# raphaelsulzer/PixelsPointsPolygons

Hardware: AMD Instinct MI355X
Metric: training tiles/sec (224px img + 3k-pt lidar) (higher is better)
Workload: dtype f32 (products as bf16x3 on the bf16 MFMA, fp32 accumulate); 1 GPU; pix2poly_fusion_s8_bs64x1; tiles_per_gpu=64, points_per_tile=3000, hip_graph=True, sync_bn=False, decoder_dropout=reference defaults (0.1 / 0.05), step=fwd+CE+10*BCE+bwd+AdamW, parallelism=dp1

## Files before the change

include/p3hip.h:

```cpp
#ifndef P3HIP_H
#define P3HIP_H
#include <stdint.h>

#ifdef __cplusplus
extern "C" {
#endif

#define P3_OK 0
#define P3_EINVAL (-1)
#define P3_ESHAPE (-2)
#define P3_EALIGN (-3)
#define P3_EUNSUP (-4)

#define P3_F32 0
#define P3_BF16 1
#define P3_F32X3 2

#define P3_ACT_NONE 0
#define P3_ACT_GELU 1
#define P3_ACT_RELU 2
#define P3_ACT_MUL 3
#define P3_ACT_BN_RELU 4

#define P3_A_PLAIN 0
#define P3_A_CONV3X3 1
#define P3_A_AFFINE_RELU 2
#define P3_A_PAIR_AFFINE_RELU 3
#define P3_A_AFFINE_MASK2 5
#define P3_A_CONV3X3_AFFINE_RELU 4

int p3_version(void);
const char* p3_last_error_string(void);
void p3_trace_kernels(int on);
const char* p3_last_kernel(void);

int p3_set_deterministic(void* scratch, int64_t bytes, int all_dtypes);
int p3_get_deterministic(void);
int p3_scratch_regions(int n);
int p3_scratch_side_stream(void* stream);
int p3_reduce_defer(float* arena, int64_t floats);
int p3_reduce_defer_enable(int on);
int p3_reduce_flush(void* stream);
int p3_reduce_pending(void);
int p3_reduce_drop(void);
int p3_scratch_stream(void* stream);
int p3_tn_defer(float* arena, int64_t floats);
int p3_tn_defer_enable(int on);
int p3_tn_flush(void* stream);
int p3_tn_pending(void);
int p3_tn_drop(void);

typedef struct {
    const unsigned long long* seed;
    unsigned int site;
    float p;
} p3_dropout;
int p3_rng_advance(unsigned long long* seed, void* stream);
int p3_transpose_many(const void* src, void* dst, const void* table, int n_entries, int total_tiles, void* stream);
int p3_dropout_apply(const void* in, int dtype_in, void* out, int dtype_out, int64_t n, int64_t ncols, const p3_dropout* drop, void* stream);

typedef struct {
    int M, N, K;
    int lda, ldb, ldc;
    int dtype_in;
    int dtype_out;
    int act;
    int a_mode;
    const float* bias;
    const void* residual;
    int ldr;
    int dtype_res;
    void* aux;
    int conv_H, conv_W, conv_C;
    const float* a_scale;
    const float* a_shift;
    const void* pair_V;
    int pair_n;
    float* colsum;
    float* colsumsq;
    p3_dropout drop;
    const void* bwd_saved;
    int bwd_act;
    float bwd_scale;
    int aux_mode;
    int conv_pad;
    const float* bwd_bn;
    const void* w_lo;
} p3_gemm_desc;
int p3_gemm(const void* A, const void* W, void* C, const p3_gemm_desc* d, void* stream);
int p3_gemm_dma(const void* A, const void* W, void* C, const p3_gemm_desc* d, int variant, void* stream);

typedef struct {
    int M, N, K;
    const void* a_hi; const void* a_lo; int lda;
    const void* w_hi; const void* w_lo; int ldb;
    void* c; void* c_lo; int ldc;
    const float* bias;
    const float* residual; int ldr;
    int act;
    float* aux; int ldaux;
    const float* mul; int ldmul;
    int tile;
    int conv_B, conv_H, conv_W, conv_ci, conv_row0;
} p3_gemm_x3_desc;
int p3_gemm_x3(const p3_gemm_x3_desc* d, void* stream);
int p3_gemm_x3_tile(int mode);
int p3_gemm_tn_x3(const void* a_hi, const void* a_lo, int lda, const void* b_hi, const void* b_lo, int ldb, float* C, int ldc, int M, int N, int K,
                  float* colsum, float* slabs, int max_slabs, void* stream);
int p3_gemm_tn_x3_conv(const void* a_hi, const void* a_lo, int lda, const void* b_hi, const void* b_lo, int ldb, float* C, int ldc, int M, int N, int Ci, int Pw,
                       float* slabs, int max_slabs, void* stream);
int p3_pad_nhwc_planes(const float* src, int ld_src, const float* pre, int ld_pre, const float* a, const float* b, void* hi, void* lo, int ld_dst, int B, int H,
                       int W, int C, int Cp, int guard, int64_t rows_total, void* stream);
int p3_col_stats(const float* x, int ld, int64_t M, int N, float* sums, float* scratch, int64_t scratch_floats, void* stream);
int p3_gemm_tn_x3_wide(int on);
int p3_to_planes(const float* src, int ld_src, void* hi, void* lo, int ld_dst, int64_t rows, int cols, void* stream);
int p3_from_planes(const void* hi, const void* lo, int ld_src, float* dst, int ld_dst, int64_t rows, int cols, void* stream);

int p3_layernorm(const void* x, const float* gamma, const float* beta, void* y, int64_t rows, int cols, int ldx, int ldy,
                 float eps, int dtype_in, int dtype_out, float* save_mean, float* save_rstd, void* stream);
int p3_layernorm_bwd_res(const void* dy, const void* x, const float* gamma, const float* mean, const float* rstd, const void* dres,
                         void* dx, float* dgamma, float* dbeta, int64_t rows, int cols, int dtype_dy, int dtype_x, int dtype_dx,
                         void* stream);
int p3_layernorm_bwd_lo(const void* dy, const void* x, const float* gamma, const float* mean, const float* rstd, const void* dres,
                        void* dx, void* dx_lo, float* dgamma, float* dbeta, int64_t rows, int cols, int dtype_dy, int dtype_x, int dtype_dx,
                        void* stream);
int p3_layernorm_bwd_lo_drop(const void* dy, const void* x, const float* gamma, const float* mean, const float* rstd, const void* dres,
                             void* dx, void* dx_lo, const p3_dropout* lo_drop, float* dgamma, float* dbeta, int64_t rows, int cols,
                             int dtype_dy, int dtype_x, int dtype_dx, void* stream);
int p3_layernorm_planes(const float* x, const float* gamma, const float* beta, void* y_hi, void* y_lo, int64_t rows, int cols, int ldx, int ldy, float eps,
                        float* save_mean, float* save_rstd, void* stream);
int p3_layernorm_bwd_planes(const float* dy, const float* x, const float* gamma, const float* mean, const float* rstd, const float* dres, float* dx,
                            void* dx_hi, void* dx_lo, int ld_planes, float* dgamma, float* dbeta, int64_t rows, int cols, void* stream);
int p3_layernorm_bwd(const void* dy, const void* x, const float* gamma, const float* mean, const float* rstd, void* dx,
                     float* dgamma, float* dbeta, int64_t rows, int cols, int dtype_dy, int dtype_x, int dtype_dx,
                     void* stream);

typedef struct {
    int B, H, Lq, Lk, head_dim;
    int64_t q_bs, k_bs, v_bs, o_bs;
    int q_rs, k_rs, v_rs, o_rs;
    float scale;
    int causal;
    const float* key_bias;
    int dtype;
    float* lse;
    p3_dropout drop;
    unsigned int* drop_rows;
    int grad_planes;
    int g_rs;
    int64_t g_bs, g_lo;
    void* o_planes;
    int op_rs;
    int64_t op_bs, op_lo;
} p3_attn_desc;
int p3_attention(const void* Q, const void* K, const void* V, void* O, const p3_attn_desc* d, void* stream);



typedef struct {
    int B;
    int64_t total_points;
    int nx, ny;
    float vx, vy, vz;
    float zmax;
    int max_points;
    int max_voxels;
    int C;
    int training;
    float bn_eps, bn_momentum;
    int dtype;
    int out_ld, out_col_off;
    int no_backward;
} p3_pillar_desc;
int64_t p3_pillar_stem_workspace_bytes(const p3_pillar_desc* d);
int p3_pillar_stem(const float* values, const int64_t* offsets, const float* w1, const float* bn1_gamma,
                   const float* bn1_beta, float* bn1_rmean, float* bn1_rvar, const void* w2, const float* bn2_gamma,
                   const float* bn2_beta, float* bn2_rmean, float* bn2_rvar, void* out, void* workspace,
                   const p3_pillar_desc* d, void* stream);
int p3_pillar_stem_layout(const p3_pillar_desc* d, int64_t* offsets);
int p3_pillar_stem_phased(const float* values, const int64_t* offsets, const float* w1, const float* bn1_gamma,
                          const float* bn1_beta, float* bn1_rmean, float* bn1_rvar, const void* w2, const float* bn2_gamma,
                          const float* bn2_beta, float* bn2_rmean, float* bn2_rvar, void* out, void* workspace,
                          const p3_pillar_desc* d, int phases, void* stream);
int p3_pillar_stem_bwd(const void* dcanvas, int dcanvas_ld, const float* w1, const float* bn1_gamma, const void* w2t,
                       const float* bn2_gamma, void* workspace, const p3_pillar_desc* d, float* dw1, float* dg1, float* db1,
                       float* dw2, float* dg2, float* db2, void* stream);
int p3_pillar_stem_bwd_phased(const void* dcanvas, int dcanvas_ld, const float* w1, const float* bn1_gamma, const void* w2t,
                              const float* bn2_gamma, void* workspace, const p3_pillar_desc* d, float* dw1, float* dg1, float* db1,
                              float* dw2, float* dg2, float* db2, const float* stat2, const float* stat1, int phases, void* stream);

int p3_patchify(const float* img, void* out, int B, int Cin, int H, int W, int P, int dtype_out, void* stream);
int p3_patchify_ld(const float* img, void* out, int B, int Cin, int H, int W, int P, int ldk, int dtype_out, void* stream);
int p3_posembed_resample(const float* table, const float* wy, const float* wx, float* out, int n_in, int n_out, int D, void* stream);
int p3_posembed_resample_bwd(const float* dout, const float* wy, const float* wx, float* dtable, int n_in, int n_out, int D, void* stream);
int p3_layerscale_fold(const float* gamma, const float* W, const float* b, float* Wf, float* bf, int N, int K, void* stream);
int p3_layerscale_fold_bwd(const float* gamma, const float* W, const float* b, const float* dWf, const float* dbf, float* dW, float* db,
                           float* dgamma, int N, int K, void* stream);
int p3_tokens_assemble(const void* src, int src_ld, int dtype_src, const float* scale, const float* shift, const float* cls,
                       const float* pos, float* x, int B, int np, int D, void* stream);
int p3_pool_pos(const void* y, int dtype_in, const float* pos, void* out, void* out_nopos, int dtype_out, int B, int np, int Din,
                int Dout, void* stream);
int p3_embed_tokens(const int64_t* tokens, const float* emb, const float* pos, void* x, float* key_bias, int B, int L, int D,
                    int pad_idx, int dtype_out, void* stream);
int p3_pair_mean(const void* feats, void* out, int B, int L, int N, int D, int dtype, void* stream);
int p3_pair_stats(const void* U, const void* V, int B, int N, int C, int dtype, float* sums, void* stream);
int p3_bn_finalize(const float* sums, int C, float count, const float* gamma, const float* beta, float* running_mean,
                   float* running_var, float eps, float momentum, int training, float* scale, float* shift, float* save_mean,
                   float* save_rstd, void* stream);
int p3_score_out(const void* H3, int dtype, const float* scale, const float* shift, const float* w4, const float* b4, float* out,
                 int B, int N, int C, int transpose_accumulate, void* stream);
int p3_sinkhorn(const float* scores, const float* alpha, int B, int m, int n, int iters, float* perm, float* z_full,
                float* uv_hist, void* stream);
int p3_assignment(const float* scores, int B, int N, int maximize, int32_t* col4row, float* perm, int32_t* status, void* stream);
int p3_argmax(const float* x, int64_t* out, int rows, int cols, int ld, void* stream);

typedef struct {
    int B, t, steps, Lmem;
    int D, H, FF;
    const void* x_in;  long long x_in_stride;
    void* x_out;       long long x_out_stride;
    void* kv_self;
    const void* kv_mem;
    const float* key_bias; long long key_bias_stride;
    const void* w_in;  const float* b_in;
    const void* w_so;  const float* b_so;
    const void* w_q;   const float* b_q;
    const void* w_co;  const float* b_co;
    const void* w1;    const float* b1;
    const void* w2;    const float* b2;
    const float *g1, *be1, *g2, *be2, *g3, *be3;
    float eps, scale;
    int cluster;
    float* exch;
    unsigned int* sync;
    int* err;
    int fp32;
} p3_decode_layer_desc;
int p3_decode_layer(const p3_decode_layer_desc* d, void* stream);
int p3_cast(const void* a, int dtype_a, void* b, int dtype_b, int64_t n, void* stream);
int p3_add_pos(const void* x, const float* pos, void* out, int B, int L, int D, int dtype, void* stream);

int p3_attention_bwd(const void* Q, const void* K, const void* V, const void* O, const void* dO, const float* lse, void* dQ,
                     void* dK, void* dV, float* delta_ws, const p3_attn_desc* d, void* stream);
int p3_gemm_tn(const void* A, const void* B, float* C, int M, int N, int K, int lda, int ldb, int ldc, int dtype, void* stream);
int p3_colsum(const void* x, float* out, int64_t M, int N, int ld, int dtype, void* stream);
int p3_act_bwd(const void* dy, int dtype_dy, const void* saved, int dtype_saved, void* out, int dtype_out, int64_t n, int act, float scale,
               void* stream);
int p3_embed_tokens_bwd(const void* dx, int dtype, const int64_t* tokens, float* demb, float* dpos, int B, int L, int D, void* stream);
int p3_embed_tokens_bwd_v(const void* dx, int dtype, const int64_t* tokens, float* demb, int B, int L, int D, int V, void* stream);
int p3_tokens_assemble_bwd(const float* dx, const void* src, int src_ld, int dtype_src, const float* scale, const float* shift, const float* mean,
                           void* dsrc, float* dscale, float* dshift, int B, int np, int D, void* stream);
int p3_pool_pos_bwd(const void* dout, int dtype_dout, void* dy, int dtype_dy, int B, int np, int Din, int Dout, void* stream);
int p3_pair_mean_bwd(const float* dF, void* dfeats, int dtype, int B, int L, int N, int D, int accumulate, void* stream);
int p3_sinkhorn_bwd(const float* scores, const float* alpha, int B, int m, int n, int iters, const float* perm,
                    const float* uv_hist, const float* dperm, float* dscores, float* dalpha, void* workspace, void* stream);
int64_t p3_sinkhorn_bwd_workspace_bytes(int B, int m, int n, int iters);
int p3_ce_loss_fwd(const float* logits, int ld, const int64_t* targets, int R, int V, int ignore_index, float* row_lse, float* acc, void* stream);
int p3_ce_loss_bwd(const float* logits, int ld, const int64_t* targets, int R, int V, int ignore_index, const float* row_lse,
                   const float* acc, const float* gscale, void* dlogits, int dtype_out, int ld_out, int Vpad, void* stream);
int p3_bce_loss_fwd(const float* p, const float* y, int64_t n, float* acc, void* stream);
int p3_bce_loss_bwd(const float* p, const float* y, int64_t n, const float* gscale, float* dp, void* stream);
int p3_adamw_schedule(long long* step, float* hyper, float base_lr, int kind, int warmup_steps, int total_steps, float beta1, float beta2,
                      void* stream);
int p3_adamw_schedule_dev(long long* step, float* hyper, const float* sched, float beta1, float beta2, void* stream);
int p3_adamw(float* params, const float* grads, float* exp_avg, float* exp_avg_sq, int64_t n, const float* hyper, float beta1,
             float beta2, float eps, float weight_decay, float grad_scale, void* bf16_shadow, void* stream);

// ... 139 lines not shown
```

pixelspointspolygons_amd/csrc/gemm_tn.hip:

```cpp
#include <stdio.h>
#include <stdlib.h>

#include <type_traits>

#include "p3_common.h"

namespace {

constexpr int TN = 128, TK = 128;

struct TnArgs {
    const void* A; const void* B; float* C;
    int M, N, K, lda, ldb, ldc, rows_per_split, tiles_k, splits;
    int Kb;
    int b_mode;
    const float* b_scale; const float* b_shift; const void* pair_V; int pair_n;
    float* slabs;
    float* colsum;
    float* cs_slab;
};

template <typename T> struct TTr;
template <> struct TTr<bf16_t> { static constexpr int BM = 64, PITCH = 160, ELEMS = 64 * 160; };
template <> struct TTr<float> { static constexpr int BM = 16, PITCH = 132, ELEMS = 16 * 132; };
// ... 350 lines not shown
            const float4 raw = *reinterpret_cast<const float4*>(p);
            a[0] += raw.x; a[1] += raw.y; a[2] += raw.z; a[3] += raw.w;
        }
    };
    if (c0 < N) {
        int64_t r = r0 + ry;
        for (; r + 3 * nrl < r1; r += 4 * nrl) {
            const T* p = x + r * ld + c0;
            add(p); add(p + (int64_t)nrl * ld); add(p + (int64_t)2 * nrl * ld); add(p + (int64_t)3 * nrl * ld);
        }
        for (; r < r1; r += nrl) add(x + r * ld + c0);
    }
#pragma unroll
    for (int k = 0; k < 4; ++k) red[ry * (ncq * 4) + q * 4 + k] = a[k];
    __syncthreads();
    if ((int)threadIdx.x < ncq * 4) {
        float s = 0.f;
        for (int y = 0; y < nrl; ++y) s += red[y * (ncq * 4) + threadIdx.x];
        const int c = blockIdx.y * 256 + threadIdx.x;
        if (c < N) {
            if (slab) slab[(int64_t)blockIdx.x * N + c] = s;
            else atomicAdd(out + c, s);
        }
    }
}

template <typename T>
__global__ __launch_bounds__(256) void colsum_scalar_kernel(const T* __restrict__ x, float* __restrict__ out, int64_t M, int N, int ld, int rows_per_block,
                                                            float* __restrict__ slab) {
    const int64_t r0 = (int64_t)blockIdx.x * rows_per_block;
    const int64_t r1 = r0 + rows_per_block < M ? r0 + rows_per_block : M;
    for (int c = threadIdx.x + blockIdx.y * 256; c < N; c += 256 * gridDim.y) {
        float s = 0.f;
        for (int64_t r = r0; r < r1; ++r) s += Cvt<T>::to_f(x[r * ld + c]);
        if (slab) slab[(int64_t)blockIdx.x * N + c] = s;
        else atomicAdd(out + c, s);
    }
}

}

void p3_tn_reduce_launch(const float* slabs, float* C, int N, int K, int ldc, int splits, hipStream_t s) {
    int64_t gr = ((int64_t)N * K + 255) / 256; if (gr > 4096) gr = 4096;
    hipLaunchKernelGGL(tn_reduce_kernel, dim3((int)gr), dim3(256), 0, s, slabs, C, N, K, ldc, splits);
}

namespace {
constexpr int TNP_MAX = 96;
struct TnpEntry { const float* slab; float* C; int N, K, ldc, splits, first_block, pad; };
struct TnpTable { TnpEntry e[TNP_MAX]; int n; };
constexpr int TNP_CAP = 4 * TNP_MAX;
TnpEntry g_tnp[TNP_CAP];
int g_tnp_n = 0, g_tnp_on = 0;
float* g_tnp_arena = nullptr;
int64_t g_tnp_cap = 0, g_tnp_used = 0;

__global__ __launch_bounds__(256) void tn_flush_kernel(TnpTable t) {
    int e = 0;
    while (e + 1 < t.n && (int)blockIdx.x >= t.e[e + 1].first_block) ++e;
    const TnpEntry en = t.e[e];
    const int64_t total = (int64_t)en.N * en.K;
    const int64_t i0 = ((int64_t)(blockIdx.x - en.first_block) * 256 + threadIdx.x) * 4;
    if (i0 >= total) return;
    double a[4] = {0.0, 0.0, 0.0, 0.0};
    int s = 0;
    for (; s + 8 <= en.splits; s += 8) {
        float4 v[8];
#pragma unroll
        for (int u = 0; u < 8; ++u) v[u] = *reinterpret_cast<const float4*>(en.slab + (int64_t)(s + u) * total + i0);
#pragma unroll
        for (int u = 0; u < 8; ++u) { a[0] += (double)v[u].x; a[1] += (double)v[u].y; a[2] += (double)v[u].z; a[3] += (double)v[u].w; }
    }
    for (; s < en.splits; ++s) {
        const float4 v = *reinterpret_cast<const float4*>(en.slab + (int64_t)s * total + i0);
        a[0] += (double)v.x; a[1] += (double)v.y; a[2] += (double)v.z; a[3] += (double)v.w;
    }
    const int n = (int)(i0 / en.K), k = (int)(i0 - (int64_t)n * en.K);
    float* c = en.C + (int64_t)n * en.ldc + k;
#pragma unroll
    for (int q = 0; q < 4; ++q) c[q] = (float)((double)c[q] + a[q]);
}
}

extern "C" int p3_tn_defer(float* arena, int64_t floats) { g_tnp_arena = arena; g_tnp_cap = arena ? floats : 0; g_tnp_used = 0; g_tnp_n = 0; return P3_OK; }
extern "C" int p3_tn_defer_enable(int on) { const int was = g_tnp_on; g_tnp_on = on ? 1 : 0; return was; }
extern "C" int p3_tn_pending(void) { return g_tnp_n; }
extern "C" int p3_tn_drop(void) { const int n = g_tnp_n; g_tnp_n = 0; g_tnp_used = 0; return n; }

float* p3_tn_park(float* C, int N, int K, int ldc, int splits) {
    const int64_t floats = (int64_t)splits * N * K;
    if (!g_tnp_on || !g_tnp_arena || g_tnp_n >= TNP_CAP || g_tnp_used + floats > g_tnp_cap || K % 4 != 0 || ldc % 4 != 0 || ((uintptr_t)C % 16) != 0) return nullptr;
    {
        const uintptr_t lo = (uintptr_t)C, hi = (uintptr_t)(C + (int64_t)(N - 1) * ldc + K);
        for (int i = 0; i < g_tnp_n; ++i) {
            const TnpEntry& o = g_tnp[i];
            const uintptr_t olo = (uintptr_t)o.C, ohi = (uintptr_t)(o.C + (int64_t)(o.N - 1) * o.ldc + o.K);
            if (lo < ohi && olo < hi) {
                if (o.ldc == ldc) {
                    const bool fwd = C >= o.C;
                    const int64_t dist = fwd ? C - o.C : o.C - C;
                    const int64_t cs = dist % ldc;
                    const int k_first = fwd ? o.K : K, k_second = fwd ? K : o.K;
                    if (cs >= k_first && cs + k_second <= ldc) continue;
                }
                return nullptr;
            }
        }
    }
    float* slot = g_tnp_arena + g_tnp_used;
    g_tnp_used += (floats + 63) / 64 * 64;
    TnpEntry& en = g_tnp[g_tnp_n++];
    en.slab = slot; en.C = C; en.N = N; en.K = K; en.ldc = ldc; en.splits = splits; en.first_block = 0; en.pad = 0;
    return slot;
}

extern "C" int p3_tn_flush(void* stream) {
    hipStream_t s = (hipStream_t)stream;
    for (int base = 0; base < g_tnp_n; base += TNP_MAX) {
        TnpTable t;
        t.n = g_tnp_n - base < TNP_MAX ? g_tnp_n - base : TNP_MAX;
        int blocks = 0;
        for (int i = 0; i < t.n; ++i) {
            t.e[i] = g_tnp[base + i];
            t.e[i].first_block = blocks;
            blocks += p3_ceil_div((int64_t)t.e[i].N * t.e[i].K, 1024);
        }
        hipLaunchKernelGGL(tn_flush_kernel, dim3(blocks), dim3(256), 0, s, t);
    }
    g_tnp_n = 0; g_tnp_used = 0;
    P3_LAUNCH_CHECK();
    return P3_OK;
}

extern "C" int p3_gemm_tn_ex(const void* A, const void* B, float* C, int M, int N, int K, int lda, int ldb, int ldc, int dtype_in, int b_mode,
                             const float* b_scale, const float* b_shift, const void* pair_V, int pair_n, float* colsum, float* slabs, int max_slabs, void* stream) {
    const bool split = dtype_in == P3_F32X3;
    const int dtype = split ? P3_F32 : dtype_in;
    P3_CHECK(A && B && C && M > 0 && N > 0 && K > 0, P3_EINVAL, "p3_gemm_tn: bad arguments");
    P3_CHECK(b_mode == 0 || b_mode == P3_A_AFFINE_RELU || b_mode == P3_A_PAIR_AFFINE_RELU || b_mode == P3_A_AFFINE_MASK2, P3_EINVAL, "p3_gemm_tn: b_mode");
    P3_CHECK(b_mode != P3_A_AFFINE_MASK2 || ldc >= 2 * K, P3_ESHAPE, "p3_gemm_tn: P3_A_AFFINE_MASK2 writes [N, 2K]");
    P3_CHECK(b_mode != P3_A_AFFINE_MASK2 || K % 8 == 0, P3_ESHAPE, "p3_gemm_tn: P3_A_AFFINE_MASK2 needs K % 8 == 0 (a staged vector must not straddle the two generated operands)");
    P3_CHECK(b_mode == 0 || (b_scale && b_shift), P3_EINVAL, "p3_gemm_tn: generated B operand needs b_scale / b_shift");
    P3_CHECK(b_mode != P3_A_PAIR_AFFINE_RELU || (pair_V && pair_n > 0 && M % (pair_n * pair_n) == 0), P3_ESHAPE, "p3_gemm_tn: pair mode needs V and M == B*n*n");
    P3_CHECK(dtype == P3_F32 || dtype == P3_BF16, P3_EUNSUP, "p3_gemm_tn: dtype");
    const int vec = dtype == P3_BF16 ? 8 : 4;
    P3_CHECK(N % vec == 0 && K % vec == 0 && lda % vec == 0 && ldb % vec == 0, P3_EALIGN, "p3_gemm_tn: N, K, lda, ldb must be multiples of 8 (bf16) / 4 (f32)");
    P3_CHECK(((uintptr_t)A % 16) == 0 && ((uintptr_t)B % 16) == 0, P3_EALIGN, "p3_gemm_tn: 16-byte base alignment");
    {
        const bool bf = dtype == P3_BF16, gen = (bf || split) && !colsum;
        hipStream_t hs = (hipStream_t)stream;
        int rc = P3_SKIP;
        if (bf && b_mode == 0)
            rc = p3_gemm_tn_dma_try(A, B, C, M, N, K, lda, ldb, ldc, colsum, slabs, max_slabs, hs);
        else if (gen && b_mode == P3_A_PAIR_AFFINE_RELU)
            rc = (bf ? p3_pair_dw_try : p3_pair_dw_x3_try)(A, B, C, M, N, K, lda, ldb, ldc, b_scale, b_shift, pair_V, pair_n, slabs, max_slabs, hs);
        else if (gen && b_mode == P3_A_AFFINE_MASK2)
            rc = (bf ? p3_mask2_dw_try : p3_mask2_dw_x3_try)(A, B, C, M, N, K, lda, ldb, ldc, b_scale, b_shift, slabs, max_slabs, hs);
        if (rc != P3_SKIP) return rc;
    }
    TnArgs g; g.A = A; g.B = B; g.C = C; g.M = M; g.N = N; g.K = K; g.lda = lda; g.ldb = ldb; g.ldc = ldc;
    g.Kb = K;
    if (b_mode == P3_A_AFFINE_MASK2) { K *= 2; g.K = K; }
    g.b_mode = b_mode; g.b_scale = b_scale; g.b_shift = b_shift; g.pair_V = pair_V; g.pair_n = pair_n; g.colsum = colsum;
    const int tiles_n = p3_ceil_div(N, TN);
    g.tiles_k = p3_ceil_div(K, TK);
    const int tiles = tiles_n * g.tiles_k;
    const int bm = dtype == P3_BF16 ? 64 : 16;
    const int tgt = 448;
    int splits = (512 % tiles == 0) ? 512 / tiles : p3_ceil_div(tgt, tiles);
    if (tgt <= 512 && splits > 1 && splits * tiles > 512) --splits;
    if (slabs && splits > max_slabs) splits = max_slabs;
    int max_splits = p3_ceil_div(M, 4 * bm);
    if (splits > max_splits) splits = max_splits;
    if (splits < 1) splits = 1;
    g.rows_per_split = p3_ceil_div(p3_ceil_div(M, splits), bm) * bm;
    splits = p3_ceil_div(M, g.rows_per_split);
    g.slabs = (slabs && splits > 1) ? slabs : nullptr;
    bool parked = false;
    if (g.slabs) { float* slot = p3_tn_park(C, N, K, ldc, splits); if (slot) { g.slabs = slot; parked = true; } }
    g.splits = splits;
    int cs_parked = 0;
    g.cs_slab = colsum ? p3_colsum_parts(splits, N, colsum, dtype, &cs_parked) : nullptr;
    dim3 grid(tiles * splits), block(256);
    hipStream_t s = (hipStream_t)stream;
#define P3_TN_LAUNCH(MODE)                                                                            \
    do {                                                                                              \
        if (dtype == P3_BF16) hipLaunchKernelGGL((gemm_tn_kernel<bf16_t, MODE>), grid, block, 0, s, g); \
        else if (split) hipLaunchKernelGGL((gemm_tn_kernel<float, MODE, true>), grid, block, 0, s, g); \
        else hipLaunchKernelGGL((gemm_tn_kernel<float, MODE>), grid, block, 0, s, g);                  \
    } while (0)
    if (p3_tracing()) {
        char nm[64];
        snprintf(nm, sizeof(nm), "gemm_tn_kernel<%s, %d>", dtype == P3_BF16 ? "bf16" : "float", g.b_mode);
        p3_note_kernel(nm);
    }
    if (g.b_mode == 0) P3_TN_LAUNCH(0);
    else if (g.b_mode == P3_A_AFFINE_RELU) P3_TN_LAUNCH(P3_A_AFFINE_RELU);
    else if (g.b_mode == P3_A_AFFINE_MASK2) P3_TN_LAUNCH(P3_A_AFFINE_MASK2);
    else P3_TN_LAUNCH(P3_A_PAIR_AFFINE_RELU);
#undef P3_TN_LAUNCH
    if (g.slabs && !parked) {
        int64_t gr = ((int64_t)N * K + 255) / 256; if (gr > 4096) gr = 4096;
        hipLaunchKernelGGL(tn_reduce_kernel, dim3((int)gr), dim3(256), 0, s, g.slabs, C, N, K, ldc, splits);
    }
    P3_LAUNCH_CHECK();
    if (g.cs_slab && !cs_parked) return p3_det_reduce(g.cs_slab, splits, N, colsum, N, 1, s);
    return P3_OK;
}

extern "C" int p3_gemm_tn(const void* A, const void* B, float* C, int M, int N, int K, int lda, int ldb, int ldc, int dtype, void* stream) {
    return p3_gemm_tn_ex(A, B, C, M, N, K, lda, ldb, ldc, dtype, 0, nullptr, nullptr, nullptr, 0, nullptr, nullptr, 0, stream);
}

extern "C" int p3_colsum(const void* x, float* out, int64_t M, int N, int ld, int dtype, void* stream) {
    P3_CHECK(x && out && M >= 0 && N > 0, P3_EINVAL, "p3_colsum: bad arguments");
    P3_CHECK(dtype == P3_BF16 || dtype == P3_F32, P3_EUNSUP, "p3_colsum: dtype");
    if (M == 0) return P3_OK;
    hipStream_t s = (hipStream_t)stream;
    const int es = dtype == P3_BF16 ? 2 : 4;
    const bool vec = (N % 4 == 0) && (ld % 4 == 0) && ((uintptr_t)x % (4 * es) == 0);
    int rpb = M > 16384 ? 128 : (M > 2048 ? 32 : 8);
    if (vec) {
        int ncq = 64;
        if (N < 256) { const int nq = (N + 3) / 4; ncq = 1; while (ncq < nq) ncq <<= 1; }
        const int cols_blocks = p3_ceil_div(N, 256);
        const int64_t want = 2048 / cols_blocks > 0 ? 2048 / cols_blocks : 1;
        const int64_t r = (M + want - 1) / want;
        if (r > rpb) rpb = (int)r;
        dim3 grid(p3_ceil_div(M, rpb), cols_blocks), block(256);
        float* slab = p3_det_scratch((int64_t)grid.x * N, dtype);
        if (dtype == P3_BF16) hipLaunchKernelGGL((colsum_kernel<bf16_t>), grid, block, 0, s, (const bf16_t*)x, out, M, N, ld, rpb, ncq, slab);
        else hipLaunchKernelGGL((colsum_kernel<float>), grid, block, 0, s, (const float*)x, out, M, N, ld, rpb, ncq, slab);
        P3_LAUNCH_CHECK();
        if (slab) return p3_det_reduce(slab, (int)grid.x, N, out, N, 1, s);
        return P3_OK;
    }
    dim3 grid(p3_ceil_div(M, rpb), p3_ceil_div(N, 256)), block(256);
    float* slab = p3_det_scratch((int64_t)grid.x * N, dtype);
    {
        if (dtype == P3_BF16) hipLaunchKernelGGL((colsum_scalar_kernel<bf16_t>), grid, block, 0, s, (const bf16_t*)x, out, M, N, ld, rpb, slab);
        else hipLaunchKernelGGL((colsum_scalar_kernel<float>), grid, block, 0, s, (const float*)x, out, M, N, ld, rpb, slab);
    }
    P3_LAUNCH_CHECK();
    if (slab) return p3_det_reduce(slab, (int)grid.x, N, out, N, 1, s);
    return P3_OK;
}
```

pixelspointspolygons_amd/csrc/p3_common.h:

```cpp
#pragma once
#include <hip/hip_runtime.h>
#include <stdint.h>
#include <stdio.h>
#include <string.h>
#include <type_traits>

#include "../../include/p3hip.h"
#include "gfx950_asm.h"

typedef uint16_t bf16_t;

typedef float f32x16 __attribute__((ext_vector_type(16)));
typedef float f32x4 __attribute__((ext_vector_type(4)));
typedef short s16x8 __attribute__((ext_vector_type(8)));
typedef short s16x4 __attribute__((ext_vector_type(4)));

__device__ __forceinline__ float bf2f(bf16_t v) { return __uint_as_float(((uint32_t)v) << 16); }
typedef float p3_f32x2 __attribute__((ext_vector_type(2)));
typedef __bf16 p3_bf16x2 __attribute__((ext_vector_type(2)));
__device__ __forceinline__ bf16_t f2bf(float f) { return __builtin_bit_cast(bf16_t, (__bf16)f); }
__device__ __forceinline__ uint32_t pack_bf2(float lo, float hi) {
    const p3_f32x2 f = {lo, hi};
    return __builtin_bit_cast(uint32_t, __builtin_convertvector(f, p3_bf16x2));
}
// ... 47 lines not shown
        const T s = red[i];
        tot = MAX ? (s > tot ? s : tot) : tot + s;
        if (i < w) base = MAX ? (s > base ? s : base) : base + s;
    }
    __syncthreads();
    total = tot;
    if (w == 0) return v;
    return MAX ? (base > v ? base : v) : base + v;
}

__device__ __forceinline__ uint32_t p3_hash32(uint32_t x) {
    x ^= x >> 16; x *= 0x7feb352du; x ^= x >> 15; x *= 0x846ca68bu; x ^= x >> 16;
    return x;
}
struct DropKey { uint32_t k0, k1, thresh; float inv_keep; bool on; };
__device__ __forceinline__ DropKey drop_key(const p3_dropout& dr) {
    DropKey k; k.on = dr.seed != nullptr && dr.p > 0.f; k.k0 = 0; k.k1 = 0; k.thresh = 0; k.inv_keep = 1.f;
    if (k.on) {
        const unsigned long long s = *dr.seed;
        k.k0 = p3_hash32((uint32_t)s ^ (dr.site * 0x9E3779B9u));
        k.k1 = p3_hash32((uint32_t)(s >> 32) + dr.site * 0x85EBCA6Bu + 0x1234567u);
        k.thresh = (uint32_t)(dr.p * 65536.f + 0.5f);
        if (k.thresh > 65535u) k.thresh = 65535u;
        k.inv_keep = 65536.f / (float)(65536u - k.thresh);
    }
    return k;
}
__device__ __forceinline__ uint32_t drop_rowkey(const DropKey& k, uint64_t row) {
    return (uint32_t)row * 0x9E3779B1u + (uint32_t)(row >> 32) * 0x7FEB352Du + k.k0;
}
__device__ __forceinline__ uint32_t drop_colkey(const DropKey& k, uint32_t col) { return (col >> 1) * 0x85EBCA77u + k.k1; }
__device__ __forceinline__ uint32_t drop_bits(uint32_t rowkey, uint32_t colkey) { return p3_hash32(rowkey ^ colkey); }
__device__ __forceinline__ bool drop_keep_lo(const DropKey& k, uint32_t bits) { return (bits & 0xffffu) >= k.thresh; }
__device__ __forceinline__ bool drop_keep_hi(const DropKey& k, uint32_t bits) { return (bits >> 16) >= k.thresh; }
__device__ __forceinline__ bool drop_keep(const DropKey& k, uint64_t row, uint32_t col) {
    const uint32_t bits = drop_bits(drop_rowkey(k, row), drop_colkey(k, col));
    return (col & 1u) ? drop_keep_hi(k, bits) : drop_keep_lo(k, bits);
}

__device__ __forceinline__ int xcd_remap(int bid, int nwg) {
    const int q = nwg / 8, r = nwg % 8, xcd = bid % 8, idx = bid / 8;
    return (xcd < r ? xcd * (q + 1) : r * (q + 1) + (xcd - r) * q) + idx;
}

__device__ __forceinline__ void attn_block_of(int lid, int nblk, int L, int pairs, int mode, int& blk, int& pair) {
    if (mode == 1 && nblk > 1 && (L & 127) != 0 && (pairs & 7) == 0) {
        const int p8 = pairs >> 3, per_xcd = p8 * nblk;
        const int x = lid / per_xcd, local = lid - x * per_xcd;
        if (local < p8) { pair = x * p8 + local; blk = nblk - 1; }
        else { const int l2 = local - p8; pair = x * p8 + l2 / (nblk - 1); blk = l2 % (nblk - 1); }
    } else { blk = lid % nblk; pair = lid / nblk; }
}
int p3_attn_order(void);

__device__ __forceinline__ int crow32(int r, int hi) { return (r & 3) + 8 * (r >> 2) + 4 * hi; }

__device__ __forceinline__ void gelu_and_grad(float x, float& h, float& g) {
    const float z = x * 0.70710678118654752440f;
    const float az = fabsf(z);
    const float t = __builtin_amdgcn_rcpf(fmaf(0.3275911f, az, 1.0f));
    const float e = __expf(-z * z);
    const float poly = t * fmaf(t, fmaf(t, fmaf(t, fmaf(t, 1.061405429f, -1.453152027f), 1.421413741f), -0.284496736f), 0.254829592f);
    const float erf_abs = fmaf(-poly, e, 1.0f);
    const float cdf = 0.5f * (1.0f + copysignf(erf_abs, z));
    h = x * cdf;
    g = fmaf(x * 0.39894228040143267794f, e, cdf);
}
__device__ __forceinline__ float gelu_erf(float x) { float h, g; gelu_and_grad(x, h, g); return h; }

__device__ __forceinline__ void p3_commit(float* out, float* slab, int n, int idx, float v) {
    if (slab) slab[(int64_t)blockIdx.x * n + idx] = v;
    else atomicAdd(out + idx, v);
}

static inline int p3_ceil_div(int64_t a, int64_t b) { return (int)((a + b - 1) / b); }
static inline int64_t p3_up256(int64_t v) { return (v + 255) & ~(int64_t)255; }

void p3_set_error(const char* msg);
int p3_tracing(void);
void p3_note_kernel(const char* name);
float* p3_det_scratch(int64_t floats, int dtype);
int p3_det_reduce(const float* parts, int nparts, int64_t stride, float* out, int nvals, int accumulate, hipStream_t s);
float* p3_reduce_scratch(int64_t floats);
float* p3_reduce_park(int64_t floats, int nparts, int nvals, int split, float* out, float* out2);
float* p3_colsum_parts(int splits, int N, float* colsum, int dtype, int* parked);
int p3_det_reduce2(const float* parts, int nparts, int64_t stride, float* tmp, float* out, float* out2, int split, int nvals, int accumulate, hipStream_t s);
#define P3_CHECK(cond, code, msg) \
    do {                          \
        if (!(cond)) {            \
            p3_set_error(msg);    \
            return (code);        \
        }                         \
    } while (0)
#define P3_LAUNCH_CHECK()                              \
    do {                                               \
        hipError_t e_ = hipGetLastError();             \
        if (e_ != hipSuccess) {                        \
            p3_set_error(hipGetErrorString(e_));       \
            return (int)e_;                            \
        }                                              \
    } while (0)

template <typename T> struct p3_type { using type = T; };
template <typename F>
static inline int p3_by_dtype(int dtype, bool x3_is_f32, const char* who, F&& f) {
    if (dtype == P3_BF16) return f(p3_type<bf16_t>{});
    if (dtype == P3_F32 || (dtype == P3_F32X3 && x3_is_f32)) return f(p3_type<float>{});
    char msg[96];
    snprintf(msg, sizeof(msg), "%s: dtype", who);
    p3_set_error(msg);
    return P3_EUNSUP;
}
template <typename T> constexpr const char* p3_dtype_name() { return sizeof(T) == sizeof(bf16_t) ? "bf16" : "float"; }
template <typename T, typename T2 = void>
static inline const char* p3_kname(const char* kernel) {
    if (!p3_tracing()) return nullptr;
    static thread_local char s[96];
    if constexpr (!__is_same(T2, void)) snprintf(s, sizeof(s), "%s<%s, %s>", kernel, p3_dtype_name<T>(), p3_dtype_name<T2>());
    else snprintf(s, sizeof(s), "%s<%s>", kernel, p3_dtype_name<T>());
    return s;
}

constexpr int P3_LAUNCH_DEVICES = 16;
template <auto Kernel, typename... Args>
static inline int p3_launch(const char* name, dim3 grid, dim3 block, size_t lds, hipStream_t s, Args... args) {
    hipError_t e = hipSuccess;
    if (lds > 64 * 1024) {
        static int raised[P3_LAUNCH_DEVICES];
        int dev = -1;
        e = hipGetDevice(&dev);
        const bool known = e == hipSuccess && dev >= 0 && dev < P3_LAUNCH_DEVICES;
        if (e == hipSuccess && !(known && raised[dev] >= (int)lds)) {
            e = hipFuncSetAttribute((const void*)Kernel, hipFuncAttributeMaxDynamicSharedMemorySize, (int)lds);
            if (e == hipSuccess && known) raised[dev] = (int)lds;
        }
    }
    if (e == hipSuccess) {
        if (name && p3_tracing()) p3_note_kernel(name);
        hipLaunchKernelGGL(Kernel, grid, block, lds, s, args...);
        e = hipGetLastError();
    }
    if (e != hipSuccess) { p3_set_error(hipGetErrorString(e)); return (int)e; }
    return P3_OK;
}

#define P3_SKIP 0x7fffffff
static_assert(P3_SKIP > 0xffff && P3_EUNSUP < 0, "P3_SKIP lies outside the P3_E* codes (negative) and the hipError_t values (small positive)");
int p3_rows_gemm_try(const void* A, const void* W, void* C, const p3_gemm_desc* d, hipStream_t s);
int p3_pair_fwd_try(const void* U, const void* W, void* C, const p3_gemm_desc* d, hipStream_t s);
int p3_pair_fwd_x3_try(const void* U, const void* W, void* C, const p3_gemm_desc* d, hipStream_t s);
int p3_rows_x3_try(const void* A, const void* W, void* C, const p3_gemm_desc* d, hipStream_t s);
int p3_gemm_tn_dma_try(const void* A, const void* B, float* C, int M, int N, int K, int lda, int ldb, int ldc, float* colsum, float* slabs, int max_slabs,
                       hipStream_t s);
int p3_pair_dw_try(const void* A, const void* U, float* C, int M, int N, int K, int lda, int ldb, int ldc, const float* scale, const float* shift,
                   const void* pair_V, int pair_n, float* slabs, int max_slabs, hipStream_t s);
int p3_pair_dw_x3_try(const void* A, const void* U, float* C, int M, int N, int K, int lda, int ldb, int ldc, const float* scale, const float* shift,
                      const void* pair_V, int pair_n, float* slabs, int max_slabs, hipStream_t s);
int p3_mask2_dw_try(const void* A, const void* B, float* C, int M, int N, int Kb, int lda, int ldb, int ldc, const float* scale, const float* shift,
                    float* slabs, int max_slabs, hipStream_t s);
int p3_mask2_dw_x3_try(const void* A, const void* B, float* C, int M, int N, int Kb, int lda, int ldb, int ldc, const float* scale, const float* shift,
                       float* slabs, int max_slabs, hipStream_t s);
void p3_tn_reduce_launch(const float* slabs, float* C, int N, int K, int ldc, int splits, hipStream_t s);
float* p3_tn_park(float* C, int N, int K, int ldc, int splits);
void p3_pair_dv_reduce_launch(const float* slab, float* dV, int nblk, int B, int N, int C, hipStream_t s);
int p3_gemm_dma_eligible(const p3_gemm_desc* d, const void* A, const void* W, const void* C);
int p3_gemm_dma_launch(const void* A, const void* W, void* C, const p3_gemm_desc* d, int variant, hipStream_t s);
bool p3_gemm_x3_as_ok(const p3_gemm_x3_desc* d);
bool p3_gemm_x3_as_default(const p3_gemm_x3_desc* d);
int p3_gemm_x3_as(const p3_gemm_x3_desc* d, hipStream_t s);
```

Before: 984.9 tiles/s.

## Add DMA-pipelined split-x3 TN weight-gradient GEMM with in-LDS bf16 plane conversion

Adds a new kernel for f32x3 TN GEMMs (weight gradients) with small N/K tile counts. It streams fp32 A and B tiles into LDS with async DMA across a 4-buffer, 3-ahead pipeline. Each tile is split into hi/lo bf16 planes in place in LDS and fed to 32x32x16 MFMAs through transposed LDS reads. Column sums are fused in and reduction uses parked slabs, replacing the generic tn path for these shapes at the cost of added code and the lossy x3 split done on the fly.

```diff
diff --git a/include/p3hip.h b/include/p3hip.h
--- a/include/p3hip.h
+++ b/include/p3hip.h
@@ -113,6 +113,7 @@
                        int W, int C, int Cp, int guard, int64_t rows_total, void* stream);
 int p3_col_stats(const float* x, int ld, int64_t M, int N, float* sums, float* scratch, int64_t scratch_floats, void* stream);
 int p3_gemm_tn_x3_wide(int on);
+int p3_gemm_tn_park(int on);
 int p3_to_planes(const float* src, int ld_src, void* hi, void* lo, int ld_dst, int64_t rows, int cols, void* stream);
 int p3_from_planes(const void* hi, const void* lo, int ld_src, float* dst, int ld_dst, int64_t rows, int cols, void* stream);
 
diff --git a/pixelspointspolygons_amd/csrc/gemm_tn.hip b/pixelspointspolygons_amd/csrc/gemm_tn.hip
--- a/pixelspointspolygons_amd/csrc/gemm_tn.hip
+++ b/pixelspointspolygons_amd/csrc/gemm_tn.hip
@@ -526,6 +526,8 @@
         int rc = P3_SKIP;
         if (bf && b_mode == 0)
             rc = p3_gemm_tn_dma_try(A, B, C, M, N, K, lda, ldb, ldc, colsum, slabs, max_slabs, hs);
+        else if (split && b_mode == 0)
+            rc = p3_gemm_tn_park_try(A, B, C, M, N, K, lda, ldb, ldc, colsum, slabs, max_slabs, hs);
         else if (gen && b_mode == P3_A_PAIR_AFFINE_RELU)
             rc = (bf ? p3_pair_dw_try : p3_pair_dw_x3_try)(A, B, C, M, N, K, lda, ldb, ldc, b_scale, b_shift, pair_V, pair_n, slabs, max_slabs, hs);
         else if (gen && b_mode == P3_A_AFFINE_MASK2)
diff --git a/pixelspointspolygons_amd/csrc/gemm_tn_park_x3.hip b/pixelspointspolygons_amd/csrc/gemm_tn_park_x3.hip
--- /dev/null
+++ b/pixelspointspolygons_amd/csrc/gemm_tn_park_x3.hip
@@ -0,0 +1,216 @@
+#include <stdlib.h>
+
+#include "p3_common.h"
+
+namespace {
+
+constexpr int TP_BM = 32;
+constexpr int TP_NBUF = 4, TP_LA = 3;
+constexpr int TP_OP = TP_BM * 128 * 4;
+constexpr int TP_BUF = 2 * TP_OP;
+constexpr int TP_LDS = TP_NBUF * TP_BUF;
+constexpr int TP_MIN_M = 128, TP_MAX_TILES = 12;
+
+struct TpArgs {
+    const float* A; const float* B; float* C;
+    int M, N, K, lda, ldb, ldc, rows_per_split, tiles_k, splits;
+    float* slabs;
+    float* colsum;
+    float* cs_slab;
+};
+
+typedef short s16x4_t __attribute__((ext_vector_type(4)));
+typedef short s16x8_t __attribute__((ext_vector_type(8)));
+typedef __attribute__((address_space(3))) s16x4_t* lds_s16x4_ptr;
+
+struct TpSet { s16x4_t ah[2], al[2], bh[2][2], bl[2][2]; };
+
+__device__ __forceinline__ bf16x8_t tp_frag(const s16x4_t& a, const s16x4_t& b) {
+    return __builtin_bit_cast(bf16x8_t, s16x8_t{a[0], a[1], a[2], a[3], b[0], b[1], b[2], b[3]});
+}
+
+__global__ __launch_bounds__(512, 2) void gemm_tn_park_x3_kernel(TpArgs g) {
+    extern __shared__ __attribute__((aligned(1024))) unsigned char lds[];
+    const int tid = threadIdx.x, lane = tid & 63, wave = __builtin_amdgcn_readfirstlane(tid >> 6), l31 = lane & 31, hi = lane >> 5;
+    const int wm = wave >> 1, wn = wave & 1;
+    const int lid = xcd_remap(blockIdx.x, gridDim.x);
+    const int tiles_all = gridDim.x / g.splits;
+    const int tile = lid % tiles_all, split = lid / tiles_all;
+    const int tn = tile / g.tiles_k, tk = tile - tn * g.tiles_k;
+    const int m_beg = split * g.rows_per_split;
+    const int m_end = min(g.M, m_beg + g.rows_per_split);
+    const int nsteps = (m_end - m_beg + TP_BM - 1) / TP_BM;
+    const uint32_t lds_addr = __builtin_amdgcn_readfirstlane((uint32_t)(uintptr_t)lds);
+
+    const int prow = lane >> 4, srow = wave * 4 + prow, ck = (lane & 15) ^ (prow << 2);
+    const float* Atile = g.A + tn * 128;
+    const float* Btile = g.B + tk * 128;
+    auto stage = [&](int st) __attribute__((always_inline)) {
+        const int m0 = m_beg + st * TP_BM;
+        const int rr = min(srow, m_end - 1 - m0);
+        const uint32_t va = (uint32_t)((rr * g.lda + ck * 8) * 4), vb = (uint32_t)((rr * g.ldb + ck * 8) * 4);
+        const uint32_t dst = lds_addr + (uint32_t)((st % TP_NBUF) * TP_BUF + wave * 2048);
+        lds_dma16x2(Atile + (int64_t)m0 * g.lda, dst, va, va + 16u);
+        lds_dma16x2(Btile + (int64_t)m0 * g.ldb, dst + (uint32_t)TP_OP, vb, vb + 16u);
+    };
+    const bool do_cs = g.colsum != nullptr && tk == 0;
+    float csum[8];
+#pragma unroll
+    for (int q = 0; q < 8; ++q) csum[q] = 0.f;
+    auto landed = [&](int ahead) __attribute__((always_inline)) {
+        if (ahead <= 0) wait_vm<0>();
+        else if (ahead == 1) wait_vm<4>();
+        else wait_vm<8>();
+    };
+    auto convert = [&](int st) __attribute__((always_inline)) {
+        unsigned char* base = lds + (st % TP_NBUF) * TP_BUF + wave * 2048 + lane * 16;
+        const bool live = m_beg + st * TP_BM + srow < m_end;
+#pragma unroll
+        for (int op = 0; op < 2; ++op) {
+            unsigned char* p = base + op * TP_OP;
+            const float4 x0 = *reinterpret_cast<const float4*>(p), x1 = *reinterpret_cast<const float4*>(p + 1024);
+            float x[8] = {x0.x, x0.y, x0.z, x0.w, x1.x, x1.y, x1.z, x1.w};
+#pragma unroll
+            for (int q = 0; q < 8; ++q) x[q] = live ? x[q] : 0.f;
+            if (op == 0 && do_cs) {
+#pragma unroll
+                for (int q = 0; q < 8; ++q) csum[q] += x[q];
+            }
+            u32x4_t h, l;
+            split8(x, h, l);
+            *reinterpret_cast<u32x4_t*>(p) = h;
+            *reinterpret_cast<u32x4_t*>(p + 1024) = l;
+        }
+    };
+
+    f32x16 acc[2];
+#pragma unroll
+    for (int j = 0; j < 2; ++j)
+#pragma unroll
+        for (int r = 0; r < 16; ++r) acc[j][r] = 0.f;
+    const int g4 = lane >> 4, li = lane & 15;
+    auto troff = [&](int ib, int hh) __attribute__((always_inline)) {
+        const int row = (g4 >> 1) * 8 + hh * 4 + (li >> 2);
+        const int slot = ib * 4 + (g4 & 1) * 2 + ((li & 3) >> 1);
+        return (uint32_t)((row >> 2) * 2048 + (row & 3) * 256 + ((slot ^ ((row & 3) << 2)) * 16) + ((li & 3) & 1) * 8);
+    };
+    uint32_t offA[2], offB[2][2];
+#pragma unroll
+    for (int hh = 0; hh < 2; ++hh) {
+        offA[hh] = troff(wm, hh);
+#pragma unroll
+        for (int j = 0; j < 2; ++j) offB[j][hh] = (uint32_t)TP_OP + troff(wn * 2 + j, hh);
+    }
+
+#pragma unroll
+    for (int p = 0; p < TP_LA; ++p)
+        if (p < nsteps) stage(p);
+    landed(min(TP_LA - 1, nsteps - 1));
+    convert(0);
+    for (int st = 0; st < nsteps; ++st) {
+        lds_barrier();
+        if (st + TP_LA < nsteps) stage(st + TP_LA);
+        const unsigned char* ab = lds + (st % TP_NBUF) * TP_BUF;
+        auto rdset = [&](int kk, TpSet& f) __attribute__((always_inline)) {
+#pragma unroll
+            for (int hh = 0; hh < 2; ++hh) {
+                const unsigned char* pa = ab + kk * 8192 + offA[hh];
+                f.ah[hh] = __builtin_amdgcn_ds_read_tr16_b64_v4i16((lds_s16x4_ptr)(pa));
+                f.al[hh] = __builtin_amdgcn_ds_read_tr16_b64_v4i16((lds_s16x4_ptr)(pa + 1024));
+#pragma unroll
+                for (int j = 0; j < 2; ++j) {
+                    const unsigned char* pb = ab + kk * 8192 + offB[j][hh];
+                    f.bh[j][hh] = __builtin_amdgcn_ds_read_tr16_b64_v4i16((lds_s16x4_ptr)(pb));
+                    f.bl[j][hh] = __builtin_amdgcn_ds_read_tr16_b64_v4i16((lds_s16x4_ptr)(pb + 1024));
+                }
+            }
+        };
+        auto block = [&](const TpSet& f) __attribute__((always_inline)) {
+            const bf16x8_t ah = tp_frag(f.ah[0], f.ah[1]), al = tp_frag(f.al[0], f.al[1]);
+            bf16x8_t bh[2], bl[2];
+#pragma unroll
+            for (int j = 0; j < 2; ++j) { bh[j] = tp_frag(f.bh[j][0], f.bh[j][1]); bl[j] = tp_frag(f.bl[j][0], f.bl[j][1]); }
+#pragma unroll
+            for (int j = 0; j < 2; ++j) acc[j] = __builtin_amdgcn_mfma_f32_32x32x16_bf16(al, bh[j], acc[j], 0, 0, 0);
+#pragma unroll
+            for (int j = 0; j < 2; ++j) acc[j] = __builtin_amdgcn_mfma_f32_32x32x16_bf16(ah, bl[j], acc[j], 0, 0, 0);
+#pragma unroll
+            for (int j = 0; j < 2; ++j) acc[j] = __builtin_amdgcn_mfma_f32_32x32x16_bf16(ah, bh[j], acc[j], 0, 0, 0);
+        };
+        TpSet f0, f1;
+        rdset(0, f0);
+        rdset(1, f1);
+        __builtin_amdgcn_sched_barrier(0);
+        block(f0);
+        __builtin_amdgcn_sched_barrier(0);
+        block(f1);
+        __builtin_amdgcn_sched_barrier(0);
+        if (st + 1 < nsteps) {
+            landed(min(TP_LA - 1, nsteps - 2 - st));
+            convert(st + 1);
+        }
+    }
+
+    if (do_cs) {
+        lds_barrier();
+        float* red = reinterpret_cast<float*>(lds);
+#pragma unroll
+        for (int q = 0; q < 8; ++q) red[(wave * 4 + prow) * 128 + ck * 8 + q] = csum[q];
+        __syncthreads();
+        if (tid < 128) {
+            float a = 0.f;
+            for (int r = 0; r < 32; ++r) a += red[r * 128 + tid];
+            if (g.cs_slab) g.cs_slab[(int64_t)split * g.N + tn * 128 + tid] = a;
+            else atomicAdd(g.colsum + tn * 128 + tid, a);
+        }
+    }
+#pragma unroll
+    for (int j = 0; j < 2; ++j) {
+        const int col = tk * 128 + (wn * 2 + j) * 32 + l31;
+        const int row0 = tn * 128 + wm * 32;
+        if (g.slabs) {
+#pragma unroll
+            for (int r = 0; r < 16; ++r) g.slabs[((int64_t)split * g.N + row0 + crow32(r, hi)) * g.K + col] = acc[j][r];
+        } else {
+#pragma unroll
+            for (int r = 0; r < 16; ++r) atomicAdd(g.C + (int64_t)(row0 + crow32(r, hi)) * g.ldc + col, acc[j][r]);
+        }
+    }
+}
+
+int g_tn_park = 1;
+
+}
+
+extern "C" int p3_gemm_tn_park(int on) { const int was = g_tn_park; g_tn_park = on ? 1 : 0; return was; }
+
+int p3_gemm_tn_park_try(const void* A, const void* B, float* C, int M, int N, int K, int lda, int ldb, int ldc, float* colsum, float* slabs, int max_slabs,
+                        hipStream_t s) {
+    if (!g_tn_park || M < TP_MIN_M || N % 128 != 0 || K % 128 != 0 || lda % 4 != 0 || ldb % 4 != 0) return P3_SKIP;
+    if (((uintptr_t)A % 16) != 0 || ((uintptr_t)B % 16) != 0) return P3_SKIP;
+    if ((int64_t)TP_BM * lda * 4 + 512 >= (1ll << 31) || (int64_t)TP_BM * ldb * 4 + 512 >= (1ll << 31)) return P3_SKIP;
+    TpArgs g;
+    g.A = (const float*)A; g.B = (const float*)B; g.C = C; g.M = M; g.N = N; g.K = K; g.lda = lda; g.ldb = ldb; g.ldc = ldc; g.colsum = colsum;
+    g.tiles_k = K / 128;
+    const int tiles = (N / 128) * g.tiles_k;
+    if (tiles > TP_MAX_TILES) return P3_SKIP;
+    int splits = 256 / tiles;
+    const int max_splits = M / (4 * TP_BM);
+    if (splits > max_splits) splits = max_splits;
+    if (slabs && splits > max_slabs) splits = max_slabs;
+    if (splits < 1) splits = 1;
+    g.rows_per_split = p3_ceil_div(p3_ceil_div(M, splits), TP_BM) * TP_BM;
+    splits = p3_ceil_div(M, g.rows_per_split);
+    g.splits = splits;
+    g.slabs = (slabs && splits > 1) ? slabs : nullptr;
+    bool parked = false;
+    if (g.slabs) { float* slot = p3_tn_park(C, N, K, ldc, splits); if (slot) { g.slabs = slot; parked = true; } }
+    int cs_parked = 0;
+    g.cs_slab = colsum ? p3_colsum_parts(splits, N, colsum, P3_F32, &cs_parked) : nullptr;
+    const int rc = p3_launch<gemm_tn_park_x3_kernel>("gemm_tn_park_x3_kernel", dim3(tiles * splits), dim3(512), TP_LDS, s, g);
+    if (rc != P3_OK) return rc;
+    if (g.slabs && !parked) p3_tn_reduce_launch(g.slabs, C, N, K, ldc, splits, s);
+    P3_LAUNCH_CHECK();
+    if (g.cs_slab && !cs_parked) return p3_det_reduce(g.cs_slab, splits, N, colsum, N, 1, s);
+    return P3_OK;
+}
diff --git a/pixelspointspolygons_amd/csrc/p3_common.h b/pixelspointspolygons_amd/csrc/p3_common.h
--- a/pixelspointspolygons_amd/csrc/p3_common.h
+++ b/pixelspointspolygons_amd/csrc/p3_common.h
@@ -223,6 +223,8 @@
 int p3_rows_x3_try(const void* A, const void* W, void* C, const p3_gemm_desc* d, hipStream_t s);
 int p3_gemm_tn_dma_try(const void* A, const void* B, float* C, int M, int N, int K, int lda, int ldb, int ldc, float* colsum, float* slabs, int max_slabs,
                        hipStream_t s);
+int p3_gemm_tn_park_try(const void* A, const void* B, float* C, int M, int N, int K, int lda, int ldb, int ldc, float* colsum, float* slabs, int max_slabs,
+                        hipStream_t s);
 int p3_pair_dw_try(const void* A, const void* U, float* C, int M, int N, int K, int lda, int ldb, int ldc, const float* scale, const float* shift,
                    const void* pair_V, int pair_n, float* slabs, int max_slabs, hipStream_t s);
 int p3_pair_dw_x3_try(const void* A, const void* U, float* C, int M, int N, int K, int lda, int ldb, int ldc, const float* scale, const float* shift,
```

Result: no change. 990.4 tiles/s (median of 6 runs) (+0.6%).
